# TencentYoutuResearch/ImageMatching-OETR

Measured on AMD Instinct MI355X. Metric: image-pairs/sec @640x640 (OETR hot path: feature correlation + overlap regression, features resident in HBM), higher is better.
Workload: dtype f32 (3xf16-split operands, fp32 accumulate); 1 GPU; BASELINE configs[1]: batch=8 pairs/GPU, 640x640 -> 20x20 tokens/image, C=256, 8 enc + 2 dec layers, f32_split_f16; pairs_per_gpu=8, global_pairs=8, streams=3, world_size=1, gpu_max_hw_queues=4, encoder_tile_rows=64, tail_mode=direct form (throughput setting for overlapped streams), parallelism=pairs sharded over 1 rank(s); all-gather of boxes only

## Files before the change

imagematching_oetr_amd/csrc/common.h:

```cpp
#pragma once
#include <hip/hip_runtime.h>
#include <stdint.h>

#include <type_traits>

namespace oetr {

constexpr int C = 256;
constexpr int NH = 8;
constexpr int HD = 32;
constexpr int FF = 512;
constexpr int TM = 32;
constexpr int LDA = C + 4;
constexpr int LDH = FF + 4;
constexpr int NTHREADS = 256;
constexpr int KV_FLOATS = NH * HD * HD;
constexpr float LN_EPS = 1e-5f;
constexpr float ATTN_EPS = 1e-6f;
constexpr int MAX_TOKENS = 10000;


#ifdef OETR_ABLATE
#define ABL(flags, bit) (((flags) & (bit)) != 0)
#else
// ... 19 lines not shown
#endif
enum { ABL_KVREDUCE = 1, ABL_GELU = 2, ABL_ELU = 4, ABL_LN = 8, ABL_GEMM = 16, ABL_STORE = 32,
       ABL_XLOAD = 64, ABL_WLOAD = 128, ABL_ATTN = 256, ABL_KVSTATE = 512 };

typedef float f32x4 __attribute__((ext_vector_type(4)));
typedef float f32x16 __attribute__((ext_vector_type(16)));
typedef _Float16 f16x8 __attribute__((ext_vector_type(8)));
typedef _Float16 f16x4 __attribute__((ext_vector_type(4)));
typedef _Float16 f16x2 __attribute__((ext_vector_type(2)));
typedef __bf16 bf16x8 __attribute__((ext_vector_type(8)));
typedef __bf16 bf16x2 __attribute__((ext_vector_type(2)));

__device__ __forceinline__ void store16(float* base_uniform, unsigned byte_off, const f32x4& v) {
  typedef uint32_t u32x4_ __attribute__((ext_vector_type(4)));
  const __amdgpu_buffer_rsrc_t rs = __builtin_amdgcn_make_buffer_rsrc(base_uniform, 0, 0x7fffffff, 0x00020000);
  __builtin_amdgcn_raw_buffer_store_b128(__builtin_bit_cast(u32x4_, v), rs, (int)byte_off, 0, 16 );
}

enum { GM_F32 = 0, GM_SPLIT = 1, GM_F16 = 2, GM_BF16 = 3 };
constexpr bool gm_half(int m) { return m != GM_F32; }
constexpr int gm_planes(int m) { return m == GM_SPLIT ? 2 : 1; }

enum { SITE_FULL = 0, SITE_ACT_HI = 1, SITE_W_HI = 2, SITE_HI = 3 };
constexpr bool site_w_lo(int s) { return s == SITE_FULL || s == SITE_ACT_HI; }
constexpr bool site_act_lo(int s) { return s == SITE_FULL || s == SITE_W_HI; }
constexpr int site_mfmas(int s) { return s == SITE_FULL ? 3 : s == SITE_HI ? 1 : 2; }
template <int POL> struct SitePolicy;
template <> struct SitePolicy<0> {
  static constexpr int Q = SITE_FULL, K = SITE_FULL, V = SITE_FULL, MERGE = SITE_FULL, MLP1 = SITE_FULL,
                       MLP2 = SITE_FULL, DEC_K = SITE_FULL, DEC_V = SITE_FULL;
};
template <> struct SitePolicy<1> {
  static constexpr int Q = SITE_HI, K = SITE_HI, V = SITE_FULL, MERGE = SITE_FULL, MLP1 = SITE_FULL,
                       MLP2 = SITE_FULL, DEC_K = SITE_HI, DEC_V = SITE_FULL;
};
constexpr int N_POLICIES = 2;

constexpr float SPLIT_SCALE = 2048.0f;
constexpr float SPLIT_INV = 1.0f / 2048.0f;
constexpr int LDAH = C + 8;
constexpr int LDHH = FF + 8;

struct Geom {
  int N;
  int L[2];
  int hf[2], wf[2];
  int nt[2];
  int row0[2];
  int prow0[2];
  int tile0[2];
  int ntiles;
  int rows;
};

#if defined(__HIPCC__)

__device__ __forceinline__ float wave_max(float v) {
#pragma unroll
  for (int off = 32; off > 0; off >>= 1) v = fmaxf(v, __shfl_xor(v, off, 64));
  return v;
}

__device__ __forceinline__ int crow(int r, int half) {
  return (r & 3) + 8 * (r >> 2) + 4 * half;
}

__device__ __forceinline__ float exp_neg(float x) {
  const float L2E_HI = 1.4426950216293335f, L2E_LO = 1.9259629911266175e-08f;
  const float t = x * L2E_HI;
  float r = fmaf(x, L2E_HI, -t);
  r = fmaf(x, L2E_LO, r);
  const float e = __builtin_amdgcn_exp2f(t);
  return fmaf(e, r * 0.69314718055994531f, e);
}
__device__ __forceinline__ float elu1(float x) {
  return __builtin_amdgcn_fmed3f(x + 1.0f, __builtin_amdgcn_exp2f(x * 1.4426950408889634f), 1.0f);
}

template <int CTRL>
__device__ __forceinline__ float dpp_mov(float v) {
  return __builtin_bit_cast(
      float, __builtin_amdgcn_update_dpp(0, __builtin_bit_cast(int, v), CTRL, 0xf, 0xf, false));
}
__device__ __forceinline__ float sum8(float v) {
  v += dpp_mov<0xB1>(v);
  v += dpp_mov<0x4E>(v);
  v += dpp_mov<0x141>(v);
  return v;
}
__device__ __forceinline__ float wave_sum(float v) {
  v = sum8(v);
  v += dpp_mov<0x140>(v);
  v += __shfl_xor(v, 16, 64);
  v += __shfl_xor(v, 32, 64);
  return v;
}
constexpr float GELU_T = 5.5f;
constexpr int GELU_DEG = 5;
constexpr float GELU_Q[GELU_DEG + 1] = {-1.151147082e+00f, -4.589156863e-01f, -5.323818670e-02f,
                                        7.977462822e-03f,  -7.398742635e-04f, 2.992419385e-05f};
__device__ __forceinline__ float gelu_erf(float x) {
  const float ax = fabsf(x), w = fminf(ax, GELU_T);
  float q = GELU_Q[GELU_DEG];
#pragma unroll
  for (int i = GELU_DEG - 1; i >= 0; --i) q = fmaf(q, w, GELU_Q[i]);
  const float e = __builtin_amdgcn_exp2f(fmaf(w, q, -1.0f));
// ... 854 lines not shown
```

imagematching_oetr_amd/csrc/encoder.hip:

```cpp
#include <type_traits>

#include "common.h"


#ifndef OETR_SOAK_AMP
#define OETR_SOAK_AMP 0
#endif
#ifndef OETR_SPLIT_STATE
#define OETR_SPLIT_STATE 1
#endif

namespace oetr {

constexpr int S0_OFF = 0;
constexpr int S1_OFF = S0_OFF + TM * LDA;
constexpr int H_OFF = S1_OFF + TILE_FLOATS;
constexpr int KSUM_OFF = H_OFF + HID_FLOATS;
constexpr int Z_OFF = KSUM_OFF + C;
constexpr int LNP_OFF = Z_OFF + TM * NH;
constexpr int SMEM_FLOATS = LNP_OFF + 6 * C;

template <int NW>
struct EncCfg {
  static constexpr int NT = 8 / NW;
// ... 651 lines not shown
    auto dec_layer = [&](auto DL) {
      constexpr int dl = decltype(DL)::value;
      constexpr int PK = dl == 0 ? P_T0 : P_T2, PV = dl == 0 ? P_T1 : P_T3;
      f32x16 accK[NT], accV[NT];
#pragma unroll
      for (int t = 0; t < NT; ++t)
#pragma unroll
        for (int r = 0; r < 16; ++r) { accK[t][r] = bias_k[dl][t]; accV[t][r] = bias_v[dl][t]; }
      ws.template gemm<C, PK, C, SP::DEC_K, SP::DEC_V>(S1, p.d.wk[dl], p.d.wk_l[dl], NT * wave, lane, accK,
                                                       p.d.wv[dl], p.d.wv_l[dl], NT * wave, p.dbg);
      ws.template gemm<C, PV, (dl == 0 ? C : 0), SP::DEC_V, SP::DEC_K>(Vin, p.d.wv[dl], p.d.wv_l[dl], NT * wave,
                                                                       lane, accV, p.d.wk[1], p.d.wk_l[1],
                                                                       NT * wave, p.dbg);
      if constexpr (dl == 1) {
        kv_state_store<MODE, NT, MASKED>(accK, accV, ABL(p.dbg, ABL_ELU), L, nvalid, lane, wave, p.dkv1_out,
                                         p.dks1_out, slot, rg, msk_s);
      } else {
#pragma unroll
        for (int t = 0; t < NT; ++t) {
          const int h = NT * wave + t;
          float ksum;
          f32x16 kv;
          kv_state_32<MODE, MASKED>(accK[t], accV[t], false, L, nvalid, half, kv, ksum, rg, msk_s);
          const float* q0 = p.dec_q0 + side * C + h * HD;
          float a = 0.f;
#pragma unroll
          for (int r = 0; r < 16; ++r) a += q0[crow(r, half)] * kv[r];
          a += __shfl_xor(a, 32, 64);
          ksum += __shfl_xor(ksum, 32, 64);
          float z = q0[col] * ksum;
          z += __shfl_xor(z, 1, 64);
          z += __shfl_xor(z, 2, 64);
          z += __shfl_xor(z, 4, 64);
          z += __shfl_xor(z, 8, 64);
          z += __shfl_xor(z, 16, 64);
          if (half == 0) p.att0_out[(size_t)slot * C + h * HD + col] = a;
          if (lane == 0) p.z0_out[(size_t)slot * NH + h] = z;
        }
      }
    };
    dec_layer(std::integral_constant<int, 0>{});
    dec_layer(std::integral_constant<int, 1>{});
  }
  range_report<MODE>(rg, p.flags);
}

constexpr int LNX_LD = 36;
template <int RTW>
struct E2 {
  static constexpr int RFL = (2 * RTW * LDAH * 2 + 3) / 4;
  static_assert(RFL >= RTW * LDA, "region holds the f32 tile too");
  static constexpr int R1 = 0, R2 = RFL, KSUM = 2 * RFL, LNP = KSUM + C;
  static constexpr int LNX = LNP + 6 * C;
  static constexpr int SMEM = LNX + RTW * LNX_LD;
};

template <int MODE, int NMT = 2, bool MASKED = false>
__device__ __forceinline__ void kv_state_64(const f32x16 (&accK)[NMT], const f32x16 (&accV)[NMT],
                                            int S_len, int nvalid, int half, bool two, f32x16& kv,
                                            float& ksum, Range& rg, const float* msk_s = nullptr) {
  const float inv_len = 1.0f / (float)S_len;
  kv = f32x16{0};
  ksum = 0.f;
  int nv2 = nvalid - 4 * half;
  asm volatile("" : "+v"(nv2));
  if constexpr (MODE == GM_SPLIT && OETR_SPLIT_STATE) {
    f32x16 c1 = {0};
#if OETR_SOAK_AMP & 2
    __builtin_amdgcn_s_setprio(3);
#endif
    auto row_tile = [&](auto MT_) {
      constexpr int mt = decltype(MT_)::value;
#pragma unroll
      for (int st = 0; st < 2; ++st) {
        f32x4 k0, k1, v0, v1;
#pragma unroll
        for (int i = 0; i < 8; ++i) {
          const int r = 8 * st + i;
          float m;
          if constexpr (MASKED) m = msk_s[32 * mt + crow(r, half)];
          else m = 32 * mt + crow(r, 0) < nv2 ? 1.0f : 0.0f;
          const float kk = elu1(accK[mt][r]) * m;
          const float vv = accV[mt][r] * (inv_len * m);
          ksum += kk;
          if (i < 4) { k0[i] = kk; v0[i] = vv; } else { k1[i - 4] = kk; v1[i - 4] = vv; }
        }
        f32x4 ah, al, bh, bl;
        split8(k0, k1, ah, al, rg);
        split8(v0, v1, bh, bl, rg);
        mma16_split3(ah, al, bh, bl, kv, c1);
        __builtin_amdgcn_sched_barrier(0);
      }
    };
    row_tile(std::integral_constant<int, 0>{});
    if constexpr (NMT == 2) {
      if (two) row_tile(std::integral_constant<int, 1>{});
    }
#if OETR_SOAK_AMP & 2
    __builtin_amdgcn_s_setprio(0);
#endif
#pragma unroll
    for (int r = 0; r < 16; ++r) kv[r] = fmaf(c1[r], SPLIT_INV, kv[r]);
  } else {
    auto row_tile = [&](auto MT_) {
      constexpr int mt = decltype(MT_)::value;
      auto operands = [&](int r, float& k, float& v) {
        float m;
        if constexpr (MASKED) m = msk_s[32 * mt + crow(r, half)];
        else m = 32 * mt + crow(r, 0) < nv2 ? 1.0f : 0.0f;
        const float x = accK[mt][r];
        k = (elu1(x)) * m;
        ksum += k;
        v = accV[mt][r] * (inv_len * m);
      };
      float kc, vc;
      operands(0, kc, vc);
#pragma unroll
      for (int r = 0; r < 16; ++r) {
        float kn = 0.f, vn = 0.f;
        if (r + 1 < 16) operands(r + 1, kn, vn);
        kv = __builtin_amdgcn_mfma_f32_32x32x2f32(kc, vc, kv, 0, 0, 0);
        __builtin_amdgcn_sched_barrier(0);
        kc = kn; vc = vn;
      }
    };
    row_tile(std::integral_constant<int, 0>{});
    if constexpr (NMT == 2) {
      if (two) row_tile(std::integral_constant<int, 1>{});
    }
  }
  ksum += __shfl_xor(ksum, 32, 64);
}
__device__ __forceinline__ void kv_state_write(const f32x16& kv, float ksum, int lane, int wave,
                                               float* __restrict__ kv_out,
                                               float* __restrict__ ks_out, int slot) {
  f32x4* dst = reinterpret_cast<f32x4*>(kv_out) + ((size_t)slot * NH + wave) * 4 * 64;
#pragma unroll
  for (int q = 0; q < 4; ++q) {
    f32x4 o = {kv[4 * q], kv[4 * q + 1], kv[4 * q + 2], kv[4 * q + 3]};
    store16(reinterpret_cast<float*>(dst), (q * 64 + (unsigned)lane) * 16u, o);
  }
  if (lane < 32) (ks_out + (size_t)slot * C + wave * HD)[(unsigned)lane] = ksum;
}

template <bool HAS_B, int TAIL, int MODE, int POL, int ROWS, int RTW = RT, bool MASKED = false>
__device__ __forceinline__ void encoder64_body(const EncLaunch& p, float* smem) {
  constexpr int NMT = RTW / 32, THREADS = 512, TPR = THREADS / RTW, F4 = 64 / TPR;
  using L2 = E2<RTW>;
  using SP = SitePolicy<POL>;
  float* R1f = smem + L2::R1;
  float* R2f = smem + L2::R2;
  Range rg;
  const PlanesT<MODE, RTW> P1(R1f, &rg), P2(R2f, &rg);
  float* Xf = HAS_B ? R2f : R1f;
  float* ksum_s = smem + L2::KSUM;
  float* lnp_s = smem + L2::LNP;
  float* lnx_s = smem + L2::LNX;
  using WS = WStream2T<MODE, ROWS, NMT>;
  WS ws;
  constexpr int P_MERGE = 0;
  constexpr int P_1A = WS::adv(P_MERGE), P_1B = WS::adv(P_1A), P_2A = WS::adv(P_1B), P_2B = WS::adv(P_2A);
  constexpr int P_T0 = HAS_B ? WS::adv(P_2B) : 0;
  constexpr int P_T1 = WS::adv(P_T0), P_T2 = WS::adv(P_T1), P_T3 = WS::adv(P_T2);

  const Geom& g = p.g;
  const int tid = threadIdx.x, lane = tid & 63, wave = __builtin_amdgcn_readfirstlane(tid >> 6);
  const int half = lane >> 5, col = lane & 31;
  const int wcol = 32 * wave;
  const int lrow = tid / TPR, lpart = tid % TPR;

  const int logical = xcd_remap(blockIdx.x, g.ntiles);
  const int per = g.nt[0] + g.nt[1];
  const int n = logical / per;
  const int rem = logical - n * per;
  const int side = rem >= g.nt[0];
  const int t_idx = side ? rem - g.nt[0] : rem;
  const int L = g.L[side];
  const int l0 = t_idx * RTW;
  const int nvalid = min(RTW, L - l0);
  const size_t row_base = (size_t)g.row0[side] + (size_t)n * L + l0;
  const int slot = g.tile0[side] + n * g.nt[side] + t_idx;
  const size_t qrow_base = (size_t)slot * RTW;
  const bool nchw = !HAS_B && p.feat_nchw[0] != nullptr;
  ws.set_rows(nvalid);
  ws.set_lane(lane);

  stage_ln_params<THREADS, HAS_B, TAIL>(lnp_s, p, tid);
  const f32x4* pos = reinterpret_cast<const f32x4*>(
                         p.pos + (size_t)(g.prow0[side] + l0 + min(lrow, nvalid - 1)) * C) + lpart;

  f32x16 xacc[NMT];
  PHASE_STAMP(p, 0);
  if (!HAS_B) PHASE_STAMP(p, 13);

  if (HAS_B) {
    const int ss = p.b_cross ? 1 - side : side;
    const int S_len = g.L[ss];
    const int nts = p.kv_reduced ? 1 : g.nt[ss];
    const int src_slot0 = p.kv_reduced ? ss * g.N + n : g.tile0[ss] + n * g.nt[ss];

    f32x4 kvB[4];
#pragma unroll
    for (int q = 0; q < 4; ++q) kvB[q] = f32x4{0.f, 0.f, 0.f, 0.f};
    {
      constexpr int KVR = 7;
      const unsigned ln = lane, kl = tid & (C - 1);
      const f32x4* kvp = reinterpret_cast<const f32x4*>(p.kv_in) + ((size_t)src_slot0 * NH + wave) * 256;
      const float* ksp = p.ks_in + (size_t)src_slot0 * C;
      float ks = 0.f;
      if (nts == 1) {
#pragma unroll
        for (int e = 0; e < 4; ++e) kvB[e] = kvp[e * 64 + ln];
        ks = ksp[kl];
      } else
      for (int ti0 = 0; ti0 < nts; ti0 += KVR) {
        f32x4 tmp[KVR][4];
        float kt[KVR];
#pragma unroll
        for (int u = 0; u < KVR; ++u) {
          const int ti = min(ti0 + u, nts - 1);
#pragma unroll
          for (int e = 0; e < 4; ++e) tmp[u][e] = kvp[(size_t)ti * (NH * 256) + e * 64 + ln];
          kt[u] = ksp[(size_t)ti * C + kl];
        }
#pragma unroll
        for (int u = 0; u < KVR; ++u)
          if (ti0 + u < nts) {
#pragma unroll
            for (int e = 0; e < 4; ++e) kvB[e] += tmp[u][e];
            ks += kt[u];
          }
      }
      if (tid < C) ksum_s[tid] = ks;
    }
    ws.template prime<C, P_MERGE, SP::MERGE>(p.b.wmerge, p.b.wmerge_l, wave, 0, lane);
    f32x4 qfrag[NMT][4];
    {
      const f32x4* qf = reinterpret_cast<const f32x4*>(p.qp + qrow_base * C) + (size_t)wave * NMT * 4 * 64;
#pragma unroll
      for (int mt = 0; mt < NMT; ++mt)
#pragma unroll
        for (int u = 0; u < 4; ++u) qfrag[mt][u] = qf[(mt * 4 + u) * 64 + (unsigned)lane];
    }
#pragma unroll
    for (int mt = 0; mt < NMT; ++mt) {
      const float* xr = p.x + (row_base + min(32 * mt + col, nvalid - 1)) * C + wcol + 4 * half;
#pragma unroll
      for (int g4 = 0; g4 < 4; ++g4) {
        const f32x4 v = *reinterpret_cast<const f32x4*>(xr + 8 * g4);
#pragma unroll
        for (int i = 0; i < 4; ++i) xacc[mt][4 * g4 + i] = v[i];
      }
    }
    __syncthreads();
    PHASE_STAMP(p, 1);

    {
      f32x4 kvh[2], kvl[2], ksh[2], ksl[2];
      const float inv_S = 1.0f / (float)S_len;
      (void)inv_S;
      if constexpr (gm_f16_range(MODE)) {
#pragma unroll
        for (int s2 = 0; s2 < 2; ++s2) {
          split8(kvB[2 * s2], kvB[2 * s2 + 1], kvh[s2], kvl[s2], rg);
          const float* kr = ksum_s + wave * HD + 4 * half + 16 * s2;
          split8(*reinterpret_cast<const f32x4*>(kr) * inv_S, *reinterpret_cast<const f32x4*>(kr + 8) * inv_S,
                 ksh[s2], ksl[s2], rg);
        }
      }
#pragma unroll
      for (int mt = 0; mt < NMT; ++mt) {
        if (mt == 1 && !ws.two()) break;
        f32x16 macc = {0}, zacc = {0};
        if constexpr (gm_f16_range(MODE)) {
          f32x16 c1 = {0}, cz = {0};
#pragma unroll
          for (int s2 = 0; s2 < 2; ++s2) {
            const f32x4 qh = qfrag[mt][2 * s2], ql = qfrag[mt][2 * s2 + 1];
            mma16_split3(kvh[s2], kvl[s2], qh, ql, macc, c1);
            mma16_split3(ksh[s2], ksl[s2], qh, ql, zacc, cz);
          }
#pragma unroll
          for (int r = 0; r < 16; ++r) macc[r] = fmaf(c1[r], SPLIT_INV, macc[r]);
          zacc[0] = fmaf(cz[0], SPLIT_INV, zacc[0]);
        } else {
#pragma unroll
          for (int ks4 = 0; ks4 < 4; ++ks4) {
            const f32x4 q = qfrag[mt][ks4];
            const f32x4 kk = *reinterpret_cast<const f32x4*>(ksum_s + wave * HD + 4 * half + ks4 * 8);
#pragma unroll
            for (int j = 0; j < 4; ++j) {
              macc = __builtin_amdgcn_mfma_f32_32x32x2f32(kvB[ks4][j], q[j], macc, 0, 0, 0);
              zacc = __builtin_amdgcn_mfma_f32_32x32x2f32(kk[j], q[j], zacc, 0, 0, 0);
            }
          }
        }
        const float zdot = gm_f16_range(MODE) ? zacc[0] * (float)S_len : zacc[0];
        const float zs = (float)S_len / (zdot + ATTN_EPS);
#pragma unroll
        for (int g4 = 0; g4 < 4; ++g4)
          P1.put4(32 * mt + col, wcol + 8 * g4 + 4 * half,
                  f32x4{macc[4 * g4] * zs, macc[4 * g4 + 1] * zs, macc[4 * g4 + 2] * zs, macc[4 * g4 + 3] * zs});
      }
    }
    __syncthreads();
    PHASE_STAMP(p, 2);

    ws.template gemm<C, P_MERGE, true, C, SP::MERGE, SP::MLP1, true>(P1, p.b.wmerge, p.b.wmerge_l, wave, 0, lane,
                                                                     xacc, p.b.w1, p.b.w1_l, wave, 0);
    PHASE_STAMP(p, 3);
    {
      float pm[NMT], pq[NMT];
#pragma unroll
      for (int mt = 0; mt < NMT; ++mt) {
        float sum = 0.f;
#pragma unroll
        for (int r = 0; r < 16; ++r) sum += xacc[mt][r];
        pm[mt] = sum * (1.0f / 16.0f);
        float q = 0.f;
#pragma unroll
        for (int r = 0; r < 16; ++r) { const float d = xacc[mt][r] - pm[mt]; q = fmaf(d, d, q); }
        pq[mt] = q;
        *reinterpret_cast<f32x2*>(lnx_s + (32 * mt + col) * LNX_LD + 2 * (2 * wave + half)) = f32x2{pm[mt], pq[mt]};
      }
      __syncthreads();
// ... 22 lines not shown
          const f32x4 gw = *reinterpret_cast<const f32x4*>(lnp_s + c0), gb = *reinterpret_cast<const f32x4*>(lnp_s + C + c0);
          f32x4 y;
#pragma unroll
          for (int i = 0; i < 4; ++i) y[i] = (xacc[mt][4 * g4 + i] - mean) * rstd * gw[i] + gb[i];
          P1.put4(32 * mt + col, c0, y);
        }
      }
    }
    __syncthreads();

    PHASE_STAMP(p, 4);
    {
      constexpr int SNEXT = TAIL == 0 ? SP::Q : SP::DEC_K;
      constexpr bool XTR = true;
      f32x16 haccA[NMT] = {}, haccB[NMT] = {};
      ws.template gemm<C, P_1A, true, C, SP::MLP1, SP::MLP1, true>(P1, p.b.w1, p.b.w1_l, wave, 0, lane, haccA,
                                                                   p.b.w1, p.b.w1_l, 8 + wave, 0);
      const bool two = ws.two();
      auto gelu_to = [&](const PlanesT<MODE, RTW>& dst, const f32x16 (&h)[NMT]) {
        return [&, two](auto CI_) {
          constexpr int CI = decltype(CI_)::value, mt = NMT == 2 ? CI / 8 : 0, g4 = NMT == 2 ? (CI % 8) / 2 : CI / 4;
          if constexpr (CI % (NMT == 2 ? 2 : 4) == 0) {
            if (mt == 1 && !two) return;
            const f32x4 ge = gelu_erf4(f32x4{h[mt][4 * g4], h[mt][4 * g4 + 1], h[mt][4 * g4 + 2], h[mt][4 * g4 + 3]});
            dst.template put4<site_act_lo(SP::MLP2)>(32 * mt + col, wcol + 8 * g4 + 4 * half, ge);
          }
        };
      };
      auto epiA = gelu_to(P2, haccA);
      ws.template gemm_epi<C, P_1B, true, FF, SP::MLP1, SP::MLP2, true>(P1, p.b.w1, p.b.w1_l, 8 + wave, 0, lane,
                                                                        haccB, p.b.w2, p.b.w2_l, wave, 0, epiA);
      __syncthreads();
      PHASE_STAMP(p, 5);
      auto epiB = gelu_to(P1, haccB);
      ws.template gemm_epi<FF, P_2A, true, FF, SP::MLP2, SP::MLP2, XTR>(P2, p.b.w2, p.b.w2_l, wave, 0, lane, xacc,
                                                                        p.b.w2, p.b.w2_l, wave, 16, epiB);
      __syncthreads();
      PHASE_STAMP(p, 6);
      PHASE_STAMP(p, 7);
      ws.template gemm<FF, P_2B, (TAIL != 2), C, SP::MLP2, SNEXT, XTR>(P1, p.b.w2, p.b.w2_l, wave, 16, lane, xacc,
                                                                       TAIL == 0 ? p.a.wq : p.d.wk[0],
                                                                       TAIL == 0 ? p.a.wq_l : p.d.wk_l[0], wave, 0);
    }
#pragma unroll
    for (int mt = 0; mt < NMT; ++mt)
#pragma unroll
      for (int g4 = 0; g4 < 4; ++g4)
        *reinterpret_cast<f32x4*>(Xf + (32 * mt + col) * LDA + wcol + 8 * g4 + 4 * half) =
            f32x4{xacc[mt][4 * g4], xacc[mt][4 * g4 + 1], xacc[mt][4 * g4 + 2], xacc[mt][4 * g4 + 3]};
    __syncthreads();
#pragma unroll
    for (int i = 0; i < RTW / 8; ++i) {
      const int r = wave + 8 * i;
      if (r < nvalid)
        store16(p.x + (row_base + r) * C, 16u * (unsigned)lane,
                                    *reinterpret_cast<const f32x4*>(Xf + r * LDA + 4 * lane));
    }
    PHASE_STAMP(p, 8);
    if (TAIL == 2) { range_report<MODE>(rg, p.flags); return; }
  } else {
    if (nchw) {
      load_tile_nchw<THREADS, RTW>(R1f, p.feat_nchw[side] + (size_t)n * C * L + l0, L, nvalid, tid);
      load_tile_nchw<THREADS, RTW>(R2f, p.pos_nchw[side] + l0, L, nvalid, tid);
    } else {
#pragma unroll
      for (int i = 0; i < (RTW * C / 4) / THREADS; ++i) {
        const int idx = tid + THREADS * i;
        const int r = idx >> 6, c4 = idx & 63;
        *reinterpret_cast<f32x4*>(R1f + r * LDA + 4 * c4) =
            reinterpret_cast<const f32x4*>(p.x + (row_base + min(r, nvalid - 1)) * C)[c4];
      }
    }
    if (TAIL == 0) ws.template prime<C, P_T0, SP::Q>(p.a.wq, p.a.wq_l, wave, 0, lane);
    if (TAIL == 1) ws.template prime<C, P_T0, SP::DEC_K>(p.d.wk[0], p.d.wk_l[0], wave, 0, lane);
    __syncthreads();
    if (nchw) {
      store_tile_tokens<THREADS, RTW>(p.x + row_base * C, R1f, nvalid, tid);
      if (n == 0) store_tile_tokens<THREADS, RTW>(p.pos_out + (size_t)(g.prow0[side] + l0) * C, R2f, nvalid, tid);
    }
    PHASE_STAMP(p, 14);
  }

  if constexpr (MASKED && TAIL != 2) {
    if (tid < RTW) lnx_s[tid] = tid < nvalid ? p.mask[side][(size_t)n * L + l0 + tid] : 0.f;
  }
  if (TAIL == 0) {
    {
      f32x4 xn[F4], ps[F4];
      if (!HAS_B && nchw) {
        const f32x4* pl = reinterpret_cast<const f32x4*>(R2f + lrow * LDA) + lpart;
#pragma unroll
        for (int i = 0; i < F4; ++i) ps[i] = pl[i * TPR];
      } else {
#pragma unroll
        for (int i = 0; i < F4; ++i) ps[i] = pos[i * TPR];
      }
      ln_rows<TPR, F4>(Xf, tid, xn, 0);
      __syncthreads();
      const f32x4* qw = reinterpret_cast<const f32x4*>(lnp_s + 2 * C) + lpart;
      const f32x4* qb = reinterpret_cast<const f32x4*>(lnp_s + 3 * C) + lpart;
      const f32x4* kw = reinterpret_cast<const f32x4*>(lnp_s + 4 * C) + lpart;
      const f32x4* kb = reinterpret_cast<const f32x4*>(lnp_s + 5 * C) + lpart;
#pragma unroll
      for (int i = 0; i < F4; ++i) {
        P1.template put4<site_act_lo(SP::Q)>(lrow, 4 * (i * TPR + lpart), (xn[i] * qw[i * TPR] + qb[i * TPR]) + ps[i]);
        P2.template put4<site_act_lo(SP::K) || site_act_lo(SP::V)>(lrow, 4 * (i * TPR + lpart),
                                                                   (xn[i] * kw[i * TPR] + kb[i * TPR]) + ps[i]);
      }
    }
    __syncthreads();
    PHASE_STAMP(p, 9);
    f32x16 accQ[NMT] = {};
    ws.template gemm<C, P_T0, true, C, SP::Q, SP::K, true>(P1, p.a.wq, p.a.wq_l, wave, 0, lane, accQ, p.a.wk,
                                                           p.a.wk_l, wave, 0);
    PHASE_STAMP(p, 10);
    f32x16 accK[NMT] = {}, accV[NMT] = {};
    {
      f32x4* qf = reinterpret_cast<f32x4*>(p.qp + qrow_base * C) + (size_t)wave * NMT * 4 * 64;
      const bool two = ws.two();
      u32x4 qhi = {0, 0, 0, 0}, qlo = {0, 0, 0, 0};
      auto qepi = [&](auto CI_) {
        constexpr int CI = decltype(CI_)::value, mt = NMT == 2 ? CI / 8 : 0, pr = NMT == 2 ? CI % 8 : CI / 2;
        constexpr int s2 = pr / 4, j = pr % 4;
        if constexpr (NMT == 1 && CI % 2 == 1) return;
        if (mt == 1 && !two) return;
        const float qmask = MASKED ? lnx_s[32 * mt + col] : 1.0f;
        const float a = MASKED ? elu1(accQ[mt][2 * pr]) * qmask : elu1(accQ[mt][2 * pr]);
        const float b = MASKED ? elu1(accQ[mt][2 * pr + 1]) * qmask : elu1(accQ[mt][2 * pr + 1]);
        if constexpr (MODE == GM_BF16) {
          if constexpr (pr % 2 == 0) { qhi[0] = __builtin_bit_cast(uint32_t, a); qhi[1] = __builtin_bit_cast(uint32_t, b); }
          else {
            qhi[2] = __builtin_bit_cast(uint32_t, a); qhi[3] = __builtin_bit_cast(uint32_t, b);
            store16(reinterpret_cast<float*>(qf), ((mt * 4 + pr / 2) * 64 + (unsigned)lane) * 16u,
                                        __builtin_bit_cast(f32x4, qhi));
          }
        } else {
          uint32_t h, l;
          cvt_planes2<GM_SPLIT>(a, b, h, l, rg);
          qhi[j] = h; qlo[j] = l;
          if constexpr (j == 3) {
            store16(reinterpret_cast<float*>(qf), ((mt * 4 + 2 * s2) * 64 + (unsigned)lane) * 16u,
                                        __builtin_bit_cast(f32x4, qhi));
            store16(reinterpret_cast<float*>(qf), ((mt * 4 + 2 * s2 + 1) * 64 + (unsigned)lane) * 16u,
                                        __builtin_bit_cast(f32x4, qlo));
          }
        }
      };
      ws.template gemm_epi<C, P_T1, true, C, SP::K, SP::V>(P2, p.a.wk, p.a.wk_l, wave, 0, lane, accK, p.a.wv,
                                                           p.a.wv_l, wave, 0, qepi);
    }
    ws.template gemm<C, P_T2, false, C, SP::V>(P2, p.a.wv, p.a.wv_l, wave, 0, lane, accV, nullptr, nullptr,
                                               0, 0);
    PHASE_STAMP(p, 11);
    f32x16 kv;
    float ksum;
    kv_state_64<MODE, NMT, MASKED>(accK, accV, L, nvalid, half, ws.two(), kv, ksum, rg, lnx_s);
    kv_state_write(kv, ksum, lane, wave, p.kv_out, p.ks_out, slot);
    PHASE_STAMP(p, 12);
  } else if (TAIL == 1) {
    float bias_k[2], bias_v[2];
#pragma unroll
    for (int dl = 0; dl < 2; ++dl) {
      bias_k[dl] = p.d.bk[dl][wcol + col];
      bias_v[dl] = p.d.bv[dl][wcol + col];
    }
    {
      f32x4 xv[F4], ps[F4];
      const f32x4* src = reinterpret_cast<const f32x4*>(Xf + lrow * LDA) + lpart;
#pragma unroll
      for (int i = 0; i < F4; ++i) { xv[i] = src[i * TPR]; ps[i] = pos[i * TPR]; }
      __syncthreads();
#pragma unroll
      for (int i = 0; i < F4; ++i) {
        P1.template put4<site_act_lo(SP::DEC_K)>(lrow, 4 * (i * TPR + lpart), xv[i] + ps[i]);
        P2.template put4<site_act_lo(SP::DEC_V)>(lrow, 4 * (i * TPR + lpart), xv[i]);
      }
    }
    __syncthreads();
    auto dec_layer = [&](auto DL) {
      constexpr int dl = decltype(DL)::value;
      constexpr int PK = dl == 0 ? P_T0 : P_T2, PV = dl == 0 ? P_T1 : P_T3;
      f32x16 accK[NMT], accV[NMT];
#pragma unroll
      for (int mt = 0; mt < NMT; ++mt)
#pragma unroll
        for (int r = 0; r < 16; ++r) { accK[mt][r] = bias_k[dl]; accV[mt][r] = bias_v[dl]; }
      ws.template gemm<C, PK, true, C, SP::DEC_K, SP::DEC_V>(P1, p.d.wk[dl], p.d.wk_l[dl], wave, 0, lane, accK,
                                                             p.d.wv[dl], p.d.wv_l[dl], wave, 0);
      ws.template gemm<C, PV, false, C, SP::DEC_V>(P2, p.d.wv[dl], p.d.wv_l[dl], wave, 0, lane, accV, nullptr,
                                                   nullptr, 0, 0);
      f32x16 kv;
      float ksum;
      kv_state_64<MODE, NMT, MASKED>(accK, accV, L, nvalid, half, ws.two(), kv, ksum, rg, lnx_s);
      if constexpr (dl == 1) {
        kv_state_write(kv, ksum, lane, wave, p.dkv1_out, p.dks1_out, slot);
      } else {
        const float* q0 = p.dec_q0 + side * C + wave * HD;
        float a = 0.f;
#pragma unroll
        for (int r = 0; r < 16; ++r) a += q0[crow(r, half)] * kv[r];
        a += __shfl_xor(a, 32, 64);
        float z = q0[col] * ksum;
        z += __shfl_xor(z, 1, 64);
        z += __shfl_xor(z, 2, 64);
        z += __shfl_xor(z, 4, 64);
        z += __shfl_xor(z, 8, 64);
        z += __shfl_xor(z, 16, 64);
        if (half == 0) p.att0_out[(size_t)slot * C + wave * HD + col] = a;
        if (lane == 0) p.z0_out[(size_t)slot * NH + wave] = z;
        ws.template prime<C, P_T2, SP::DEC_K>(p.d.wk[1], p.d.wk_l[1], wave, 0, lane);
      }
    };
    dec_layer(std::integral_constant<int, 0>{});
    dec_layer(std::integral_constant<int, 1>{});
  }
  range_report<MODE>(rg, p.flags);
}

template <bool HAS_B, int TAIL, int MODE, int POL = 0, bool MASKED = false>
__global__ __launch_bounds__(512) void k_encoder64(EncLaunch p) {
  __shared__ __attribute__((aligned(16))) float smem[E2<RT>::SMEM];
  if constexpr (gm_planes(MODE) == 2) {
    const Geom& g = p.g;
    const int logical = xcd_remap(blockIdx.x, g.ntiles);
    const int per = g.nt[0] + g.nt[1];
    const int rem = logical - (logical / per) * per;
    const int side = rem >= g.nt[0];
    const int t_idx = side ? rem - g.nt[0] : rem;
    const int nvalid = min(RT, g.L[side] - t_idx * RT);
    if (__builtin_amdgcn_readfirstlane(nvalid > 32 ? 1 : 0)) encoder64_body<HAS_B, TAIL, MODE, POL, 2, RT, MASKED>(p, smem);
    else encoder64_body<HAS_B, TAIL, MODE, POL, 1, RT, MASKED>(p, smem);
  } else {
    encoder64_body<HAS_B, TAIL, MODE, POL, 0, RT, MASKED>(p, smem);
  }
}

template <bool HAS_B, int TAIL, int MODE, int POL = 0, bool MASKED = false>
__global__ __launch_bounds__(512) void k_encoder32m(EncLaunch p) {
  __shared__ __attribute__((aligned(16))) float smem[E2<TM>::SMEM];
  encoder64_body<HAS_B, TAIL, MODE, POL, 2, TM, MASKED>(p, smem);
}

template <int NOB_TAIL_MAX, class F>
static hipError_t launch_b_tail(bool has_b, int tail, F launch) {
  constexpr std::integral_constant<int, 0> t0{};
  constexpr std::integral_constant<int, 1> t1{};
  constexpr std::integral_constant<int, 2> t2{};
  if (has_b) {
    if (tail == 0) launch(std::true_type{}, t0);
    else if (tail == 1) launch(std::true_type{}, t1);
    else launch(std::true_type{}, t2);
  } else {
    if (tail == 0) launch(std::false_type{}, t0);
    else if constexpr (NOB_TAIL_MAX == 0) return hipErrorInvalidValue;
    else if (tail == 1) launch(std::false_type{}, t1);
    else if constexpr (NOB_TAIL_MAX == 1) return hipErrorInvalidValue;
    else launch(std::false_type{}, t2);
  }
  return hipGetLastError();
}

template <int MODE>
static hipError_t launch_encoder_mode(const EncLaunch& p, bool has_b, int tail, hipStream_t s) {
  const dim3 grid(p.g.ntiles);
  if (p.mask[0] || p.mask[1]) {
    if constexpr (MODE == GM_SPLIT) {
      if (!p.mask[0] || !p.mask[1] || (p.policy != 0 && p.policy != 1) || p.attn_full) return hipErrorInvalidValue;
      return launch_b_tail<0>(has_b, tail, [&](auto b, auto t) {
        if (p.policy == 1) {
          if (p.tile_rows == RT) hipLaunchKernelGGL((k_encoder64<b(), t(), MODE, 1, true>), grid, dim3(512), 0, s, p);
          else hipLaunchKernelGGL((k_encoder32m<b(), t(), MODE, 1, true>), grid, dim3(512), 0, s, p);
        } else {
          if (p.tile_rows == RT) hipLaunchKernelGGL((k_encoder64<b(), t(), MODE, 0, true>), grid, dim3(512), 0, s, p);
          else hipLaunchKernelGGL((k_encoder32m<b(), t(), MODE, 0, true>), grid, dim3(512), 0, s, p);
        }
      });
    } else if constexpr (MODE == GM_F32) {
      if (!p.mask[0] || !p.mask[1] || p.policy != 0 || p.attn_full) return hipErrorInvalidValue;
      return launch_b_tail<0>(has_b, tail, [&](auto b, auto t) {
        hipLaunchKernelGGL((k_encoder<b(), t(), MODE, 4, false, 0, true>), grid, dim3(64 * 4), 0, s, p);
      });
    } else {
      return hipErrorInvalidValue;
    }
  }
  if constexpr (gm_half(MODE)) {
    if (p.tile_rows == RT) {
      if constexpr (MODE == GM_SPLIT) {
        if (p.policy == 1)
          return launch_b_tail<1>(has_b, tail, [&](auto b, auto t) {
            hipLaunchKernelGGL((k_encoder64<b(), t(), MODE, 1>), grid, dim3(512), 0, s, p);
          });
      }
      if (p.policy != 0) return hipErrorInvalidValue;
      return launch_b_tail<1>(has_b, tail, [&](auto b, auto t) {
        hipLaunchKernelGGL((k_encoder64<b(), t(), MODE>), grid, dim3(512), 0, s, p);
      });
    }
  }
  if constexpr (MODE == GM_SPLIT) {
    if (!p.attn_full) {
      if (p.policy != 0 && p.policy != 1) return hipErrorInvalidValue;
      return launch_b_tail<1>(has_b, tail, [&](auto b, auto t) {
        if (p.policy == 1) hipLaunchKernelGGL((k_encoder32m<b(), t(), MODE, 1>), grid, dim3(512), 0, s, p);
        else hipLaunchKernelGGL((k_encoder32m<b(), t(), MODE, 0>), grid, dim3(512), 0, s, p);
      });
    }
  }
  constexpr int NW = gm_half(MODE) ? 8 : 4;
  if (p.policy != 0) return hipErrorInvalidValue;
  if (p.attn_full) {
    if constexpr (gm_f16_range(MODE) || MODE == GM_F32) {
      return launch_b_tail<0>(has_b, tail, [&](auto b, auto t) {
        hipLaunchKernelGGL((k_encoder<b(), t(), MODE, 8, true>), grid, dim3(64 * 8), 0, s, p);
      });
    } else {
      return hipErrorInvalidValue;
    }
  }
  if constexpr (MODE != GM_SPLIT) {
    return launch_b_tail<2>(has_b, tail, [&](auto b, auto t) {
      hipLaunchKernelGGL((k_encoder<b(), t(), MODE, NW>), grid, dim3(64 * NW), 0, s, p);
    });
  }
  return hipErrorInvalidValue;
}

__global__ __launch_bounds__(256) void k_kv_reduce(Geom g, const float* __restrict__ kvp,
                                                   const float* __restrict__ ksp, float* __restrict__ kvr,
                                                   float* __restrict__ ksr) {
  const int img = blockIdx.x >> 3, head = blockIdx.x & 7, lane = threadIdx.x & 63;
  const int e = __builtin_amdgcn_readfirstlane(threadIdx.x >> 6);
  const int side = img >= g.N, n = img - side * g.N;
  const int nt = g.nt[side];
  const int slot0 = g.tile0[side] + n * nt;
  const f32x4* src = reinterpret_cast<const f32x4*>(kvp) + ((size_t)slot0 * NH + head) * 256 + e * 64 + lane;
  const float* ks = ksp + (size_t)slot0 * C + head * HD + (lane & 31);
  f32x4 acc = f32x4{0.f, 0.f, 0.f, 0.f};
  float kacc = 0.f;
  constexpr int U = 16;
  for (int t0 = 0; t0 < nt; t0 += U) {
    f32x4 tmp[U];
    float kt[U];
#pragma unroll
    for (int u = 0; u < U; ++u) {
      const int t = min(t0 + u, nt - 1);
      tmp[u] = src[(size_t)t * (NH * 256)];
      kt[u] = ks[(size_t)t * C];
    }
// ... 29 lines not shown
```

Before: 34570 image-pairs/s.

## Pack both images' partial tail tiles into one 64-row encoder workgroup

When both images' last 64-row tiles hold at most 32 valid tokens, the two tails are now handled by a single workgroup. Each tail occupies one 32-row half, and the grid shrinks by one workgroup per pair. Cross-attention state reduction, Q/X loads, stores, KV-state and decoder partials are all computed per half using that half's own geometry and slot. The aim is to remove half-empty tail workgroups and their wasted MFMA and weight-streaming work. The cost is extra code paths, more register and LDS use (a second ksum buffer), and per-row branching in the paired path.

```diff
diff --git a/imagematching_oetr_amd/csrc/common.h b/imagematching_oetr_amd/csrc/common.h
--- a/imagematching_oetr_amd/csrc/common.h
+++ b/imagematching_oetr_amd/csrc/common.h
@@ -95,6 +95,13 @@
   int ntiles;
   int rows;
 };
+#if defined(__HIPCC__)
+__host__ __device__
+#endif
+inline bool enc_pairs_tails(const Geom& g) {
+  const int t0 = g.L[0] - (g.nt[0] - 1) * 64, t1 = g.L[1] - (g.nt[1] - 1) * 64;
+  return t0 >= 1 && t0 <= 32 && t1 >= 1 && t1 <= 32;
+}
 
 #if defined(__HIPCC__)
 
diff --git a/imagematching_oetr_amd/csrc/encoder.hip b/imagematching_oetr_amd/csrc/encoder.hip
--- a/imagematching_oetr_amd/csrc/encoder.hip
+++ b/imagematching_oetr_amd/csrc/encoder.hip
@@ -727,7 +727,8 @@
   static_assert(RFL >= RTW * LDA, "region holds the f32 tile too");
   static constexpr int R1 = 0, R2 = RFL, KSUM = 2 * RFL, LNP = KSUM + C;
   static constexpr int LNX = LNP + 6 * C;
-  static constexpr int SMEM = LNX + RTW * LNX_LD;
+  static constexpr int KSUM2 = LNX + RTW * LNX_LD;
+  static constexpr int SMEM = KSUM2 + (RTW == 64 ? C : 0);
 };
 
 template <int MODE, int NMT = 2, bool MASKED = false>
@@ -806,6 +807,9 @@
   }
   ksum += __shfl_xor(ksum, 32, 64);
 }
+__device__ __forceinline__ const f32x16 (&one_tile(const f32x16& acc))[1] {
+  return *reinterpret_cast<const f32x16(*)[1]>(&acc);
+}
 __device__ __forceinline__ void kv_state_write(const f32x16& kv, float ksum, int lane, int wave,
                                                float* __restrict__ kv_out,
                                                float* __restrict__ ks_out, int slot) {
@@ -816,6 +820,21 @@
     store16(reinterpret_cast<float*>(dst), (q * 64 + (unsigned)lane) * 16u, o);
   }
   if (lane < 32) (ks_out + (size_t)slot * C + wave * HD)[(unsigned)lane] = ksum;
+}
+
+struct Enc64Tile { int n, side, t_idx; bool pair_tile; };
+constexpr bool enc64_pairable(int mode, int rtw, bool masked) { return gm_planes(mode) == 2 && rtw == 64 && !masked; }
+__device__ __forceinline__ Enc64Tile enc64_tile(const Geom& g, bool paired) {
+  const int f0 = g.nt[0] - (paired ? 1 : 0), f1 = g.nt[1] - (paired ? 1 : 0);
+  const int per = f0 + f1 + (paired ? 1 : 0);
+  const int logical = xcd_remap(blockIdx.x, paired ? g.ntiles - g.N : g.ntiles);
+  Enc64Tile t;
+  t.n = logical / per;
+  const int rem = logical - t.n * per;
+  t.pair_tile = paired && rem == f0 + f1;
+  t.side = !t.pair_tile && rem >= f0;
+  t.t_idx = t.pair_tile ? f0 : t.side ? rem - f0 : rem;
+  return t;
 }
 
 template <bool HAS_B, int TAIL, int MODE, int POL, int ROWS, int RTW = RT, bool MASKED = false>
@@ -831,7 +850,10 @@
   float* ksum_s = smem + L2::KSUM;
   float* lnp_s = smem + L2::LNP;
   float* lnx_s = smem + L2::LNX;
-  using WS = WStream2T<MODE, ROWS, NMT>;
+  constexpr bool PAIR = ROWS == 3;
+  constexpr bool PAIRABLE = enc64_pairable(MODE, RTW, MASKED);
+  static_assert(!PAIR || PAIRABLE, "pair workgroups: 64 rows, unmasked, two-plane");
+  using WS = WStream2T<MODE, PAIR ? 2 : ROWS, NMT>;
   WS ws;
   constexpr int P_MERGE = 0;
   constexpr int P_1A = WS::adv(P_MERGE), P_1B = WS::adv(P_1A), P_2A = WS::adv(P_1B), P_2B = WS::adv(P_2A);
@@ -844,12 +866,8 @@
   const int wcol = 32 * wave;
   const int lrow = tid / TPR, lpart = tid % TPR;
 
-  const int logical = xcd_remap(blockIdx.x, g.ntiles);
-  const int per = g.nt[0] + g.nt[1];
-  const int n = logical / per;
-  const int rem = logical - n * per;
-  const int side = rem >= g.nt[0];
-  const int t_idx = side ? rem - g.nt[0] : rem;
+  const Enc64Tile id = enc64_tile(g, PAIR || (PAIRABLE && enc_pairs_tails(g)));
+  const int n = id.n, side = id.side, t_idx = id.t_idx;
   const int L = g.L[side];
   const int l0 = t_idx * RTW;
   const int nvalid = min(RTW, L - l0);
@@ -859,10 +877,22 @@
   const bool nchw = !HAS_B && p.feat_nchw[0] != nullptr;
   ws.set_rows(nvalid);
   ws.set_lane(lane);
+  int L_t[2], l0_t[2], nv_t[2], slot_t[2];
+  size_t rb_t[2];
+#pragma unroll
+  for (int mt = 0; mt < 2; ++mt) {
+    L_t[mt] = g.L[mt];
+    l0_t[mt] = (g.nt[mt] - 1) * RTW;
+    nv_t[mt] = L_t[mt] - l0_t[mt];
+    rb_t[mt] = (size_t)g.row0[mt] + (size_t)n * L_t[mt] + l0_t[mt];
+    slot_t[mt] = g.tile0[mt] + n * g.nt[mt] + g.nt[mt] - 1;
+  }
 
   stage_ln_params<THREADS, HAS_B, TAIL>(lnp_s, p, tid);
+  const int pmt = lrow >> 5;
   const f32x4* pos = reinterpret_cast<const f32x4*>(
-                         p.pos + (size_t)(g.prow0[side] + l0 + min(lrow, nvalid - 1)) * C) + lpart;
+                         p.pos + (PAIR ? (size_t)(g.prow0[pmt] + l0_t[pmt] + min(lrow & 31, nv_t[pmt] - 1))
+                                       : (size_t)(g.prow0[side] + l0 + min(lrow, nvalid - 1))) * C) + lpart;
 
   f32x16 xacc[NMT];
   PHASE_STAMP(p, 0);
@@ -874,52 +904,72 @@
     const int nts = p.kv_reduced ? 1 : g.nt[ss];
     const int src_slot0 = p.kv_reduced ? ss * g.N + n : g.tile0[ss] + n * g.nt[ss];
 
-    f32x4 kvB[4];
-#pragma unroll
-    for (int q = 0; q < 4; ++q) kvB[q] = f32x4{0.f, 0.f, 0.f, 0.f};
-    {
+    constexpr int NST = PAIR ? 2 : 1;
+    int S_len_t[2];
+    f32x4 kvB_t[NST][4];
+    float* const ksum2_s = smem + L2::KSUM2;
+    auto reduce_state = [&](int slot0, int ntiles, f32x4 (&kvB)[4], float* ksum_dst) {
+#pragma unroll
+      for (int q = 0; q < 4; ++q) kvB[q] = f32x4{0.f, 0.f, 0.f, 0.f};
       constexpr int KVR = 7;
       const unsigned ln = lane, kl = tid & (C - 1);
-      const f32x4* kvp = reinterpret_cast<const f32x4*>(p.kv_in) + ((size_t)src_slot0 * NH + wave) * 256;
-      const float* ksp = p.ks_in + (size_t)src_slot0 * C;
+      const f32x4* kvp = reinterpret_cast<const f32x4*>(p.kv_in) + ((size_t)slot0 * NH + wave) * 256;
+      const float* ksp = p.ks_in + (size_t)slot0 * C;
       float ks = 0.f;
-      if (nts == 1) {
+      if (ntiles == 1) {
 #pragma unroll
         for (int e = 0; e < 4; ++e) kvB[e] = kvp[e * 64 + ln];
         ks = ksp[kl];
       } else
-      for (int ti0 = 0; ti0 < nts; ti0 += KVR) {
+      for (int ti0 = 0; ti0 < ntiles; ti0 += KVR) {
         f32x4 tmp[KVR][4];
         float kt[KVR];
 #pragma unroll
         for (int u = 0; u < KVR; ++u) {
-          const int ti = min(ti0 + u, nts - 1);
+          const int ti = min(ti0 + u, ntiles - 1);
 #pragma unroll
           for (int e = 0; e < 4; ++e) tmp[u][e] = kvp[(size_t)ti * (NH * 256) + e * 64 + ln];
           kt[u] = ksp[(size_t)ti * C + kl];
         }
 #pragma unroll
         for (int u = 0; u < KVR; ++u)
-          if (ti0 + u < nts) {
+          if (ti0 + u < ntiles) {
 #pragma unroll
             for (int e = 0; e < 4; ++e) kvB[e] += tmp[u][e];
             ks += kt[u];
           }
       }
-      if (tid < C) ksum_s[tid] = ks;
-    }
+      if (tid < C) ksum_dst[tid] = ks;
+    };
+    if constexpr (PAIR) {
+#pragma unroll
+      for (int mt = 0; mt < 2; ++mt) {
+        const int st = p.b_cross ? 1 - mt : mt;
+        S_len_t[mt] = g.L[st];
+        reduce_state(p.kv_reduced ? st * g.N + n : g.tile0[st] + n * g.nt[st], p.kv_reduced ? 1 : g.nt[st], kvB_t[mt],
+                     mt ? ksum2_s : ksum_s);
+      }
+    } else {
+      S_len_t[0] = S_len_t[1] = S_len;
+      reduce_state(src_slot0, nts, kvB_t[0], ksum_s);
+    }
+    f32x4 (&kvB)[4] = kvB_t[0];
     ws.template prime<C, P_MERGE, SP::MERGE>(p.b.wmerge, p.b.wmerge_l, wave, 0, lane);
     f32x4 qfrag[NMT][4];
     {
       const f32x4* qf = reinterpret_cast<const f32x4*>(p.qp + qrow_base * C) + (size_t)wave * NMT * 4 * 64;
 #pragma unroll
-      for (int mt = 0; mt < NMT; ++mt)
-#pragma unroll
-        for (int u = 0; u < 4; ++u) qfrag[mt][u] = qf[(mt * 4 + u) * 64 + (unsigned)lane];
+      for (int mt = 0; mt < NMT; ++mt) {
+        const f32x4* qt = PAIR ? reinterpret_cast<const f32x4*>(p.qp + (size_t)slot_t[mt] * RTW * C) + (size_t)wave * NMT * 4 * 64
+                               : qf + mt * 4 * 64;
+#pragma unroll
+        for (int u = 0; u < 4; ++u) qfrag[mt][u] = qt[u * 64 + (unsigned)lane];
+      }
     }
 #pragma unroll
     for (int mt = 0; mt < NMT; ++mt) {
-      const float* xr = p.x + (row_base + min(32 * mt + col, nvalid - 1)) * C + wcol + 4 * half;
+      const float* xr = p.x + (PAIR ? rb_t[mt] + min(col, nv_t[mt] - 1) : row_base + min(32 * mt + col, nvalid - 1)) * C +
+                        wcol + 4 * half;
 #pragma unroll
       for (int g4 = 0; g4 < 4; ++g4) {
         const f32x4 v = *reinterpret_cast<const f32x4*>(xr + 8 * g4);
@@ -932,20 +982,22 @@
 
     {
       f32x4 kvh[2], kvl[2], ksh[2], ksl[2];
-      const float inv_S = 1.0f / (float)S_len;
-      (void)inv_S;
-      if constexpr (gm_f16_range(MODE)) {
+      auto state_planes = [&](const f32x4 (&kvS)[4], const float* ksum_src, int S_src) {
+        const float inv_S = 1.0f / (float)S_src;
 #pragma unroll
         for (int s2 = 0; s2 < 2; ++s2) {
-          split8(kvB[2 * s2], kvB[2 * s2 + 1], kvh[s2], kvl[s2], rg);
-          const float* kr = ksum_s + wave * HD + 4 * half + 16 * s2;
+          split8(kvS[2 * s2], kvS[2 * s2 + 1], kvh[s2], kvl[s2], rg);
+          const float* kr = ksum_src + wave * HD + 4 * half + 16 * s2;
           split8(*reinterpret_cast<const f32x4*>(kr) * inv_S, *reinterpret_cast<const f32x4*>(kr + 8) * inv_S,
                  ksh[s2], ksl[s2], rg);
         }
-      }
+      };
+      if constexpr (gm_f16_range(MODE) && !PAIR) state_planes(kvB, ksum_s, S_len);
 #pragma unroll
       for (int mt = 0; mt < NMT; ++mt) {
         if (mt == 1 && !ws.two()) break;
+        if constexpr (PAIR) state_planes(kvB_t[mt], mt ? ksum2_s : ksum_s, S_len_t[mt]);
+        const int S_len = S_len_t[mt];
         f32x16 macc = {0}, zacc = {0};
         if constexpr (gm_f16_range(MODE)) {
           f32x16 c1 = {0}, cz = {0};
@@ -1074,6 +1126,12 @@
 #pragma unroll
     for (int i = 0; i < RTW / 8; ++i) {
       const int r = wave + 8 * i;
+      if constexpr (PAIR) {
+        const int mt = i >= 4 ? 1 : 0;
+        if (r - 32 * mt < nv_t[mt])
+          store16(p.x + (rb_t[mt] + r - 32 * mt) * C, 16u * (unsigned)lane,
+                                      *reinterpret_cast<const f32x4*>(Xf + r * LDA + 4 * lane));
+      } else
       if (r < nvalid)
         store16(p.x + (row_base + r) * C, 16u * (unsigned)lane,
                                     *reinterpret_cast<const f32x4*>(Xf + r * LDA + 4 * lane));
@@ -1081,6 +1139,23 @@
     PHASE_STAMP(p, 8);
     if (TAIL == 2) { range_report<MODE>(rg, p.flags); return; }
   } else {
+    if constexpr (PAIR) {
+      if (nchw) {
+#pragma unroll
+        for (int mt = 0; mt < 2; ++mt) {
+          load_tile_nchw<THREADS, 32>(R1f + 32 * mt * LDA, p.feat_nchw[mt] + (size_t)n * C * L_t[mt] + l0_t[mt], L_t[mt], nv_t[mt], tid);
+          load_tile_nchw<THREADS, 32>(R2f + 32 * mt * LDA, p.pos_nchw[mt] + l0_t[mt], L_t[mt], nv_t[mt], tid);
+        }
+      } else {
+#pragma unroll
+        for (int i = 0; i < (RTW * C / 4) / THREADS; ++i) {
+          const int idx = tid + THREADS * i;
+          const int r = idx >> 6, c4 = idx & 63, mt = r >> 5;
+          *reinterpret_cast<f32x4*>(R1f + r * LDA + 4 * c4) =
+              reinterpret_cast<const f32x4*>(p.x + (rb_t[mt] + min(r & 31, nv_t[mt] - 1)) * C)[c4];
+        }
+      }
+    } else
     if (nchw) {
       load_tile_nchw<THREADS, RTW>(R1f, p.feat_nchw[side] + (size_t)n * C * L + l0, L, nvalid, tid);
       load_tile_nchw<THREADS, RTW>(R2f, p.pos_nchw[side] + l0, L, nvalid, tid);
@@ -1096,6 +1171,15 @@
     if (TAIL == 0) ws.template prime<C, P_T0, SP::Q>(p.a.wq, p.a.wq_l, wave, 0, lane);
     if (TAIL == 1) ws.template prime<C, P_T0, SP::DEC_K>(p.d.wk[0], p.d.wk_l[0], wave, 0, lane);
     __syncthreads();
+    if constexpr (PAIR) {
+      if (nchw) {
+#pragma unroll
+        for (int mt = 0; mt < 2; ++mt) {
+          store_tile_tokens<THREADS, 32>(p.x + rb_t[mt] * C, R1f + 32 * mt * LDA, nv_t[mt], tid);
+          if (n == 0) store_tile_tokens<THREADS, 32>(p.pos_out + (size_t)(g.prow0[mt] + l0_t[mt]) * C, R2f + 32 * mt * LDA, nv_t[mt], tid);
+        }
+      }
+    } else
     if (nchw) {
       store_tile_tokens<THREADS, RTW>(p.x + row_base * C, R1f, nvalid, tid);
       if (n == 0) store_tile_tokens<THREADS, RTW>(p.pos_out + (size_t)(g.prow0[side] + l0) * C, R2f, nvalid, tid);
@@ -1138,7 +1222,8 @@
     PHASE_STAMP(p, 10);
     f32x16 accK[NMT] = {}, accV[NMT] = {};
     {
-      f32x4* qf = reinterpret_cast<f32x4*>(p.qp + qrow_base * C) + (size_t)wave * NMT * 4 * 64;
+      f32x4* qf0 = reinterpret_cast<f32x4*>(p.qp + qrow_base * C) + (size_t)wave * NMT * 4 * 64;
+      f32x4* qf1 = PAIR ? reinterpret_cast<f32x4*>(p.qp + (size_t)slot_t[1] * RTW * C) + (size_t)wave * NMT * 4 * 64 - 4 * 64 : qf0;
       const bool two = ws.two();
       u32x4 qhi = {0, 0, 0, 0}, qlo = {0, 0, 0, 0};
       auto qepi = [&](auto CI_) {
@@ -1149,6 +1234,7 @@
         const float qmask = MASKED ? lnx_s[32 * mt + col] : 1.0f;
         const float a = MASKED ? elu1(accQ[mt][2 * pr]) * qmask : elu1(accQ[mt][2 * pr]);
         const float b = MASKED ? elu1(accQ[mt][2 * pr + 1]) * qmask : elu1(accQ[mt][2 * pr + 1]);
+        f32x4* const qf = mt == 1 ? qf1 : qf0;
         if constexpr (MODE == GM_BF16) {
           if constexpr (pr % 2 == 0) { qhi[0] = __builtin_bit_cast(uint32_t, a); qhi[1] = __builtin_bit_cast(uint32_t, b); }
           else {
@@ -1174,10 +1260,21 @@
     ws.template gemm<C, P_T2, false, C, SP::V>(P2, p.a.wv, p.a.wv_l, wave, 0, lane, accV, nullptr, nullptr,
                                                0, 0);
     PHASE_STAMP(p, 11);
+    if constexpr (PAIR) {
+#pragma unroll
+      for (int mt = 0; mt < 2; ++mt) {
+        f32x16 kv;
+        float ksum;
+        kv_state_64<MODE, 1>(one_tile(accK[mt]), one_tile(accV[mt]), L_t[mt], nv_t[mt], half, false, kv, ksum, rg);
+        asm volatile("" : "+v"(rg.fm));
+        kv_state_write(kv, ksum, lane, wave, p.kv_out, p.ks_out, slot_t[mt]);
+      }
+    } else {
     f32x16 kv;
     float ksum;
     kv_state_64<MODE, NMT, MASKED>(accK, accV, L, nvalid, half, ws.two(), kv, ksum, rg, lnx_s);
     kv_state_write(kv, ksum, lane, wave, p.kv_out, p.ks_out, slot);
+    }
     PHASE_STAMP(p, 12);
   } else if (TAIL == 1) {
     float bias_k[2], bias_v[2];
@@ -1211,27 +1308,41 @@
                                                              p.d.wv[dl], p.d.wv_l[dl], wave, 0);
       ws.template gemm<C, PV, false, C, SP::DEC_V>(P2, p.d.wv[dl], p.d.wv_l[dl], wave, 0, lane, accV, nullptr,
                                                    nullptr, 0, 0);
-      f32x16 kv;
-      float ksum;
-      kv_state_64<MODE, NMT, MASKED>(accK, accV, L, nvalid, half, ws.two(), kv, ksum, rg, lnx_s);
-      if constexpr (dl == 1) {
-        kv_state_write(kv, ksum, lane, wave, p.dkv1_out, p.dks1_out, slot);
+      auto dec_partials = [&](const f32x16& kv, float ksum, int tside, int tslot) {
+        asm volatile("" : "+v"(rg.fm));
+        if constexpr (dl == 1) {
+          kv_state_write(kv, ksum, lane, wave, p.dkv1_out, p.dks1_out, tslot);
+        } else {
+          const float* q0 = p.dec_q0 + tside * C + wave * HD;
+          float a = 0.f;
+#pragma unroll
+          for (int r = 0; r < 16; ++r) a += q0[crow(r, half)] * kv[r];
+          a += __shfl_xor(a, 32, 64);
+          float z = q0[col] * ksum;
+          z += __shfl_xor(z, 1, 64);
+          z += __shfl_xor(z, 2, 64);
+          z += __shfl_xor(z, 4, 64);
+          z += __shfl_xor(z, 8, 64);
+          z += __shfl_xor(z, 16, 64);
+          if (half == 0) p.att0_out[(size_t)tslot * C + wave * HD + col] = a;
+          if (lane == 0) p.z0_out[(size_t)tslot * NH + wave] = z;
+        }
+      };
+      if constexpr (PAIR) {
+#pragma unroll
+        for (int mt = 0; mt < 2; ++mt) {
+          f32x16 kv;
+          float ksum;
+          kv_state_64<MODE, 1>(one_tile(accK[mt]), one_tile(accV[mt]), L_t[mt], nv_t[mt], half, false, kv, ksum, rg);
+          dec_partials(kv, ksum, mt, slot_t[mt]);
+        }
       } else {
-        const float* q0 = p.dec_q0 + side * C + wave * HD;
-        float a = 0.f;
-#pragma unroll
-        for (int r = 0; r < 16; ++r) a += q0[crow(r, half)] * kv[r];
-        a += __shfl_xor(a, 32, 64);
-        float z = q0[col] * ksum;
-        z += __shfl_xor(z, 1, 64);
-        z += __shfl_xor(z, 2, 64);
-        z += __shfl_xor(z, 4, 64);
-        z += __shfl_xor(z, 8, 64);
-        z += __shfl_xor(z, 16, 64);
-        if (half == 0) p.att0_out[(size_t)slot * C + wave * HD + col] = a;
-        if (lane == 0) p.z0_out[(size_t)slot * NH + wave] = z;
-        ws.template prime<C, P_T2, SP::DEC_K>(p.d.wk[1], p.d.wk_l[1], wave, 0, lane);
-      }
+        f32x16 kv;
+        float ksum;
+        kv_state_64<MODE, NMT, MASKED>(accK, accV, L, nvalid, half, ws.two(), kv, ksum, rg, lnx_s);
+        dec_partials(kv, ksum, side, slot);
+      }
+      if constexpr (dl == 0) ws.template prime<C, P_T2, SP::DEC_K>(p.d.wk[1], p.d.wk_l[1], wave, 0, lane);
     };
     dec_layer(std::integral_constant<int, 0>{});
     dec_layer(std::integral_constant<int, 1>{});
@@ -1244,12 +1355,15 @@
   __shared__ __attribute__((aligned(16))) float smem[E2<RT>::SMEM];
   if constexpr (gm_planes(MODE) == 2) {
     const Geom& g = p.g;
-    const int logical = xcd_remap(blockIdx.x, g.ntiles);
-    const int per = g.nt[0] + g.nt[1];
-    const int rem = logical - (logical / per) * per;
-    const int side = rem >= g.nt[0];
-    const int t_idx = side ? rem - g.nt[0] : rem;
-    const int nvalid = min(RT, g.L[side] - t_idx * RT);
+    constexpr bool PAIRABLE = enc64_pairable(MODE, RT, MASKED);
+    const Enc64Tile id = enc64_tile(g, PAIRABLE && enc_pairs_tails(g));
+    const int nvalid = min(RT, g.L[id.side] - id.t_idx * RT);
+    if constexpr (PAIRABLE) {
+      if (__builtin_amdgcn_readfirstlane(id.pair_tile ? 1 : 0)) {
+        encoder64_body<HAS_B, TAIL, MODE, POL, 3, RT, MASKED>(p, smem);
+        return;
+      }
+    }
     if (__builtin_amdgcn_readfirstlane(nvalid > 32 ? 1 : 0)) encoder64_body<HAS_B, TAIL, MODE, POL, 2, RT, MASKED>(p, smem);
     else encoder64_body<HAS_B, TAIL, MODE, POL, 1, RT, MASKED>(p, smem);
   } else {
@@ -1308,15 +1422,16 @@
   }
   if constexpr (gm_half(MODE)) {
     if (p.tile_rows == RT) {
+      const dim3 grid64(enc64_pairable(MODE, RT, false) && enc_pairs_tails(p.g) ? p.g.ntiles - p.g.N : p.g.ntiles);
       if constexpr (MODE == GM_SPLIT) {
         if (p.policy == 1)
           return launch_b_tail<1>(has_b, tail, [&](auto b, auto t) {
-            hipLaunchKernelGGL((k_encoder64<b(), t(), MODE, 1>), grid, dim3(512), 0, s, p);
+            hipLaunchKernelGGL((k_encoder64<b(), t(), MODE, 1>), grid64, dim3(512), 0, s, p);
           });
       }
       if (p.policy != 0) return hipErrorInvalidValue;
       return launch_b_tail<1>(has_b, tail, [&](auto b, auto t) {
-        hipLaunchKernelGGL((k_encoder64<b(), t(), MODE>), grid, dim3(512), 0, s, p);
+        hipLaunchKernelGGL((k_encoder64<b(), t(), MODE>), grid64, dim3(512), 0, s, p);
       });
     }
   }
```

Result: no change. 34410 image-pairs/s (-0.5%).
